# hikvision-research/ProbabilisticTeacher

Hardware: AMD Instinct MI355X
Metric: teacher-student train-step img/s at 1333x800 (higher is better)
Workload: dtype f32; 1 GPU; BASELINE configs[2]: final_c2f.yaml (K=8) full teacher+student+EMA step, per-GPU 16 labelled + 16 unlabelled synthetic 1333x800 images, BURN_UP_STEP=0, random init; global_batch=32, parallelism=dp1

## Files before the change

### probabilisticteacher_amd/csrc/nms.hip

```cpp
#include "common.h"

namespace {

typedef unsigned long long u64;

__device__ __forceinline__ int seg_count(const int32_t* __restrict__ seg, const int32_t* __restrict__ cnt, int img)
{
    const int cap = seg[img + 1] - seg[img];
    return cnt ? min(cap, cnt[img]) : cap;
}

__global__ __launch_bounds__(64) void nms_mask_kernel(const float* __restrict__ boxes,
                                                      const int32_t* __restrict__ seg,
                                                      const int32_t* __restrict__ cnt, float thr, int words,
                                                      int64_t max_count, u64* __restrict__ mask)
{
    const int cb = blockIdx.x, rb = blockIdx.y, img = blockIdx.z;
    if (cb < rb) return;
    const int beg = seg[img], n = seg_count(seg, cnt, img);
    if (rb * 64 >= n || cb * 64 >= n) return;
    __shared__ float4 cbox[64];
    __shared__ float carea[64];
    const int t = threadIdx.x;
    const int cj = cb * 64 + t;
    if (cj < n) {
        const float4 b = reinterpret_cast<const float4*>(boxes)[beg + cj];
        cbox[t] = b;
        carea[t] = (b.z - b.x) * (b.w - b.y);
    }
    __syncthreads();
    const int i = rb * 64 + t;
    if (i >= n) return;
    const float4 a = reinterpret_cast<const float4*>(boxes)[beg + i];
    const float aarea = (a.z - a.x) * (a.w - a.y);
    const int lim = min(64, n - cb * 64);
    u64 bits = 0;
    const int start = (cb == rb) ? t + 1 : 0;
    constexpr float HI = 1.f + 0x1p-20f, LO = 1.f - 0x1p-20f;
    for (int k = start; k < lim; ++k) {
        const float4 b = cbox[k];
        const float xx1 = fmaxf(a.x, b.x), yy1 = fmaxf(a.y, b.y);
        const float xx2 = fminf(a.z, b.z), yy2 = fminf(a.w, b.w);
        float w = xx2 - xx1, h = yy2 - yy1;
        w = w < 0.f ? 0.f : w;
        h = h < 0.f ? 0.f : h;
        const float inter = w * h;
        const float uni = aarea + carea[k] - inter;
        const float p = thr * uni;
        bool sup;
        if (uni > 0.f && p >= 1.17549435e-38f && inter > p * HI) sup = true;
        else if (uni > 0.f && p >= 1.17549435e-38f && inter < p * LO) sup = false;
        else sup = inter / uni > thr;
        if (sup) bits |= 1ull << k;
    }
    mask[((size_t)img * max_count + i) * words + cb] = bits;
}

constexpr int SCAN_THREADS = 256;

__global__ __launch_bounds__(SCAN_THREADS) void nms_scan_kernel(const u64* __restrict__ mask, const int32_t* __restrict__ seg,
                                                                const int32_t* __restrict__ cnt, int words, int64_t max_count,
                                                                int max_keep, int32_t* __restrict__ keep,
                                                                int32_t* __restrict__ keep_count)
{
    extern __shared__ u64 removed[];
    __shared__ u64 kept_s;
    __shared__ int count_s;
    const int img = blockIdx.x, tid = threadIdx.x, lane = tid & 63;
    const int wave = __builtin_amdgcn_readfirstlane(tid >> 6);
    const int n = seg_count(seg, cnt, img);
    const u64* M = mask + (size_t)img * max_count * words;
    for (int w = tid; w < words; w += SCAN_THREADS) removed[w] = 0;
    if (tid == 0) count_s = 0;
    __syncthreads();
    int count = 0;
    const int chunks = (n + 63) / 64;
    u64 diag_next = (wave == 0 && lane < n) ? M[(size_t)lane * words] : 0;
    for (int c = 0; c < chunks; ++c) {
        if (wave == 0) {
            const int row = c * 64 + lane;
            const u64 diag = diag_next;
            if (c + 1 < chunks) {
                const int rn = row + 64;
                diag_next = (rn < n) ? M[(size_t)rn * words + c + 1] : 0;
            }
            u64 cur = removed[c];
            if (c == chunks - 1 && (n & 63)) cur |= ~0ull << (n & 63);
            u64 alive = ~(((u64)(unsigned)__builtin_amdgcn_readfirstlane((int)(unsigned)(cur >> 32)) << 32) |
                          (u64)(unsigned)__builtin_amdgcn_readfirstlane((int)(unsigned)cur));
            u64 kept = 0;
            const unsigned dlo = (unsigned)diag, dhi = (unsigned)(diag >> 32);
            while (alive) {
                const int i = __builtin_ctzll(alive);
                kept |= 1ull << i;
                const u64 di = ((u64)(unsigned)__builtin_amdgcn_readlane((int)dhi, i) << 32) |
                               (u64)(unsigned)__builtin_amdgcn_readlane((int)dlo, i);
                alive &= ~(di | (1ull << i));
            }
            if ((kept >> lane) & 1ull) {
                const int pos = count + __popcll(kept & ((1ull << lane) - 1ull));
                if (pos < max_keep) keep[(size_t)img * max_keep + pos] = row;
            }
            if (lane == 0) {
                kept_s = kept;
                count_s = count + __popcll(kept);
            }
        }
        __syncthreads();
        count = count_s;
        if (count >= max_keep) break;
        const unsigned klo = (unsigned)__builtin_amdgcn_readfirstlane((int)(unsigned)kept_s);
        const unsigned khi = (unsigned)__builtin_amdgcn_readfirstlane((int)(unsigned)(kept_s >> 32));
        const u64 kept = ((u64)khi << 32) | klo;
        for (int w = c + 1 + tid; w < chunks; w += SCAN_THREADS) {
            u64 acc = removed[w];
            const u64* Mw = M + (size_t)c * 64 * words + w;
            u64 k = kept;
            while (k) {
                u64 v[16];
#pragma unroll
                for (int j = 0; j < 16; ++j) {
                    if (k) {
                        const int i = __builtin_ctzll(k);
                        k &= k - 1;
                        v[j] = Mw[(size_t)i * words];
                    } else v[j] = 0ull;
                }
#pragma unroll
                for (int j = 0; j < 16; ++j) acc |= v[j];
            }
            removed[w] = acc;
        }
        __syncthreads();
    }
    if (tid == 0) keep_count[img] = count < max_keep ? count : max_keep;
}

}

extern "C" {

int64_t ptmi_nms_ws_bytes(int64_t max_count, int nimg)
{
    const int64_t words = (max_count + 63) / 64;
    return (int64_t)nimg * max_count * words * 8;
}

int ptmi_nms_batched(const float* boxes, const int32_t* seg_offsets, const int32_t* seg_counts, int nimg,
                     int64_t max_count, float thr, int max_keep, int32_t* keep_out, int32_t* keep_count, void* ws,
                     ptmi_stream_t s)
{
    PTMI_CHECK_ARG(seg_offsets && keep_out && keep_count && nimg > 0 && max_count >= 0 && max_keep > 0,
                   "nms_batched: bad args");
    PTMI_CHECK_ARG(max_count == 0 || (boxes && ws), "nms_batched: boxes / workspace missing");
    hipStream_t st = (hipStream_t)s;
    if (max_count == 0) {
        hipError_t e = hipMemsetAsync(keep_count, 0, sizeof(int32_t) * (size_t)nimg, st);
        if (e != hipSuccess) { ptmi_set_error("nms_batched: memset failed"); return -2; }
        return 0;
    }
    const int words = (int)((max_count + 63) / 64);
    PTMI_CHECK_ARG((size_t)words * 8 <= 64 * 1024, "nms_batched: max_count %lld too large", (long long)max_count);
    dim3 grid(words, words, nimg);
    hipLaunchKernelGGL(nms_mask_kernel, grid, dim3(64), 0, st, boxes, seg_offsets, seg_counts, thr, words, max_count,
                       reinterpret_cast<u64*>(ws));
    PTMI_LAUNCH_CHECK("nms_mask");
    hipLaunchKernelGGL(nms_scan_kernel, dim3(nimg), dim3(SCAN_THREADS), (size_t)words * 8, st, reinterpret_cast<const u64*>(ws),
                       seg_offsets, seg_counts, words, max_count, max_keep, keep_out, keep_count);
    PTMI_LAUNCH_CHECK("nms_scan");
    return 0;
}

}
```

Before: 95.65 img/s.

## Process NMS in row bands with early exit once max_keep reached

Splits the NMS mask and scan into bands of 32 chunks (2048 boxes). Each band computes only its rows of the IoU mask, then scans them, saving the removed bitmask and keep count to global state. Later bands are skipped per image once max_keep is reached, so mask work for low-score boxes is avoided. This adds kernel launches per band and a global round-trip of the removed state.

Result: no change. 96.64 img/s, median of 4 (+1.0%).

```diff
diff --git a/probabilisticteacher_amd/csrc/nms.hip b/probabilisticteacher_amd/csrc/nms.hip
--- a/probabilisticteacher_amd/csrc/nms.hip
+++ b/probabilisticteacher_amd/csrc/nms.hip
@@ -3,6 +3,16 @@
 namespace {
 
 typedef unsigned long long u64;
+
+#ifndef PTMI_NMS_BAND_CHUNKS
+#define PTMI_NMS_BAND_CHUNKS 32
+#endif
+constexpr int NMS_BAND_CHUNKS = PTMI_NMS_BAND_CHUNKS;
+
+struct NmsState {
+    int32_t count;
+    int32_t done;
+};
 
 __device__ __forceinline__ int seg_count(const int32_t* __restrict__ seg, const int32_t* __restrict__ cnt, int img)
 {
@@ -13,10 +23,12 @@
 __global__ __launch_bounds__(64) void nms_mask_kernel(const float* __restrict__ boxes,
                                                       const int32_t* __restrict__ seg,
                                                       const int32_t* __restrict__ cnt, float thr, int words,
-                                                      int64_t max_count, u64* __restrict__ mask)
-{
-    const int cb = blockIdx.x, rb = blockIdx.y, img = blockIdx.z;
+                                                      int64_t max_count, int rb0, const NmsState* __restrict__ state,
+                                                      u64* __restrict__ mask)
+{
+    const int cb = rb0 + blockIdx.x, rb = rb0 + blockIdx.y, img = blockIdx.z;
     if (cb < rb) return;
+    if (state && state[img].done) return;
     const int beg = seg[img], n = seg_count(seg, cnt, img);
     if (rb * 64 >= n || cb * 64 >= n) return;
     __shared__ float4 cbox[64];
@@ -60,27 +72,31 @@
 
 __global__ __launch_bounds__(SCAN_THREADS) void nms_scan_kernel(const u64* __restrict__ mask, const int32_t* __restrict__ seg,
                                                                 const int32_t* __restrict__ cnt, int words, int64_t max_count,
-                                                                int max_keep, int32_t* __restrict__ keep,
-                                                                int32_t* __restrict__ keep_count)
+                                                                int max_keep, int c0, int cend,
+                                                                u64* __restrict__ removed_g, NmsState* __restrict__ state,
+                                                                int32_t* __restrict__ keep, int32_t* __restrict__ keep_count)
 {
     extern __shared__ u64 removed[];
     __shared__ u64 kept_s;
     __shared__ int count_s;
     const int img = blockIdx.x, tid = threadIdx.x, lane = tid & 63;
     const int wave = __builtin_amdgcn_readfirstlane(tid >> 6);
+    if (c0 > 0 && state[img].done) return;
     const int n = seg_count(seg, cnt, img);
     const u64* M = mask + (size_t)img * max_count * words;
-    for (int w = tid; w < words; w += SCAN_THREADS) removed[w] = 0;
-    if (tid == 0) count_s = 0;
+    u64* R = removed_g + (size_t)img * words;
+    const int chunks = (n + 63) / 64;
+    const int cl = min(chunks, cend);
+    for (int w = c0 + tid; w < chunks; w += SCAN_THREADS) removed[w] = c0 > 0 ? R[w] : 0ull;
+    int count = c0 > 0 ? state[img].count : 0;
+    if (tid == 0) count_s = count;
     __syncthreads();
-    int count = 0;
-    const int chunks = (n + 63) / 64;
-    u64 diag_next = (wave == 0 && lane < n) ? M[(size_t)lane * words] : 0;
-    for (int c = 0; c < chunks; ++c) {
+    u64 diag_next = (wave == 0 && c0 * 64 + lane < n) ? M[(size_t)(c0 * 64 + lane) * words + c0] : 0;
+    for (int c = c0; c < cl; ++c) {
         if (wave == 0) {
             const int row = c * 64 + lane;
             const u64 diag = diag_next;
-            if (c + 1 < chunks) {
+            if (c + 1 < cl) {
                 const int rn = row + 64;
                 diag_next = (rn < n) ? M[(size_t)rn * words + c + 1] : 0;
             }
@@ -133,7 +149,18 @@
         }
         __syncthreads();
     }
-    if (tid == 0) keep_count[img] = count < max_keep ? count : max_keep;
+    if (count >= max_keep || cl >= chunks) {
+        if (tid == 0) {
+            keep_count[img] = count < max_keep ? count : max_keep;
+            state[img].done = 1;
+        }
+        return;
+    }
+    for (int w = cl + tid; w < chunks; w += SCAN_THREADS) R[w] = removed[w];
+    if (tid == 0) {
+        state[img].count = count;
+        state[img].done = 0;
+    }
 }
 
 }
@@ -143,7 +170,7 @@
 int64_t ptmi_nms_ws_bytes(int64_t max_count, int nimg)
 {
     const int64_t words = (max_count + 63) / 64;
-    return (int64_t)nimg * max_count * words * 8;
+    return (int64_t)nimg * max_count * words * 8 + (int64_t)nimg * words * 8 + (int64_t)nimg * sizeof(NmsState);
 }
 
 int ptmi_nms_batched(const float* boxes, const int32_t* seg_offsets, const int32_t* seg_counts, int nimg,
@@ -161,13 +188,19 @@
     }
     const int words = (int)((max_count + 63) / 64);
     PTMI_CHECK_ARG((size_t)words * 8 <= 64 * 1024, "nms_batched: max_count %lld too large", (long long)max_count);
-    dim3 grid(words, words, nimg);
-    hipLaunchKernelGGL(nms_mask_kernel, grid, dim3(64), 0, st, boxes, seg_offsets, seg_counts, thr, words, max_count,
-                       reinterpret_cast<u64*>(ws));
-    PTMI_LAUNCH_CHECK("nms_mask");
-    hipLaunchKernelGGL(nms_scan_kernel, dim3(nimg), dim3(SCAN_THREADS), (size_t)words * 8, st, reinterpret_cast<const u64*>(ws),
-                       seg_offsets, seg_counts, words, max_count, max_keep, keep_out, keep_count);
-    PTMI_LAUNCH_CHECK("nms_scan");
+    u64* mask = reinterpret_cast<u64*>(ws);
+    u64* removed = mask + (size_t)nimg * max_count * words;
+    NmsState* state = reinterpret_cast<NmsState*>(removed + (size_t)nimg * words);
+    for (int c0 = 0; c0 < words; c0 += NMS_BAND_CHUNKS) {
+        const int cend = min(c0 + NMS_BAND_CHUNKS, words);
+        dim3 grid(words - c0, cend - c0, nimg);
+        hipLaunchKernelGGL(nms_mask_kernel, grid, dim3(64), 0, st, boxes, seg_offsets, seg_counts, thr, words, max_count, c0,
+                           c0 > 0 ? state : (const NmsState*)nullptr, mask);
+        PTMI_LAUNCH_CHECK("nms_mask");
+        hipLaunchKernelGGL(nms_scan_kernel, dim3(nimg), dim3(SCAN_THREADS), (size_t)words * 8, st, (const u64*)mask, seg_offsets,
+                           seg_counts, words, max_count, max_keep, c0, cend, removed, state, keep_out, keep_count);
+        PTMI_LAUNCH_CHECK("nms_scan");
+    }
     return 0;
 }
 
```
